# ziniuwan/maed

Measured on AMD Instinct MI355X. Metric: video-clips/sec (BxT frames) train step, higher is better.
Workload: dtype bf16

## Files before the change

### include/maed_hip.h

```cpp
#ifndef MAED_HIP_H
#define MAED_HIP_H

#include <stddef.h>
#include <stdint.h>

#ifdef __cplusplus
extern "C" {
#endif

typedef enum { MAED_F32 = 0, MAED_BF16 = 1,
               MAED_F32X3 = 2, MAED_F32X6 = 3,
               MAED_F32X1 = 4 } maed_dtype;

typedef enum {
    MAED_OK = 0,
    MAED_ERR_ARG = -1,
    MAED_ERR_SHAPE = -2,
    MAED_ERR_ALIGN = -3,
    MAED_ERR_LAUNCH = -4,
    MAED_ERR_UNSUPPORTED = -5
} maed_status;

typedef enum {
    MAED_EPI_STORE = 0,
// ... 17 lines not shown

const char* maed_last_error(void);
int maed_version(void);

typedef enum {
    MAED_OPT_F32_MATMUL = 0,
    MAED_OPT_SIDE_STREAM = 1,
    MAED_OPT_TN_TARGET_WGS = 2,
    MAED_OPT_ABLATE = 3,
    MAED_OPT_GN_BWD_ONEPASS = 4,
    MAED_OPT_F32_BWD_X1 = 5,
    MAED_OPT_ST_FUSED = 6,
    MAED_OPT_CONV3X3_ROWS_WGS = 7,
    MAED_OPT_STEM_WGRAD_WGS = 8,
    MAED_OPT_LBS_FRAMES = 9,
    MAED_OPT_TN_DMA = 10,
    MAED_OPT_X3_PLANES = 11,
    MAED_OPT_X3_PLANES_LN = 12,
    MAED_OPT_SK = 13,
    MAED_OPT_SK_GRID = 14,
    MAED_OPT_TN_SK = 15,
    MAED_OPT_CONV3X3_NARROW_WGS = 16,
    MAED_OPT_CONV3X3_FRAME = 17,
    MAED_OPT_COUNT
} maed_option;
int maed_init(int device);
int maed_device_faults(void);
int maed_device_faults_clear(void);
int maed_set_option(int key, int value);
int maed_get_option(int key);

int maed_layernorm_fwd(const float* x, int64_t x_row_stride, const float* gamma, const float* beta,
                       void* y, int dtype, float* mean, float* rstd,
                       int64_t rows, int C, float eps, void* stream);
int maed_layernorm_bwd(const void* dy, int dtype, const float* x, int64_t x_row_stride,
                       const float* gamma, const float* mean, const float* rstd,
                       const float* dres_in, float* dx_out, void* dx_twin, float* dgamma, float* dbeta,
                       int64_t rows, int C, void* stream);

int maed_gemm_nt(const void* A, int64_t lda, const void* B, int64_t ldb,
                 int64_t M, int64_t N, int64_t K, int dtype, int epilogue,
                 const float* bias, void* out, int64_t ldo, void* out2,
                 const void* aux, int64_t ldaux, int splitk, int impl, void* stream);

int maed_gemm_nt_planes(const void* a_hi, const void* a_lo, int64_t lda, const void* b_hi, const void* b_lo, int64_t ldb, int64_t M, int64_t N, int64_t K,
                        int epilogue, const float* bias, void* out, int64_t ldo, void* out2_bf16, const void* aux, int64_t ldaux, void* out_hi, void* out_lo,
// ... 157 lines not shown
int maed_groupnorm_fwd_twin(const void* x, const void* residual, const float* gamma, const float* beta, void* y, double* sums,
                            uint8_t* relu_mask, int N, int HW, int C, float eps, int relu, int sums_zeroed, void* twin_x, void* twin_y, void* stream);
#define MAED_GN_SYNC_WORDS 80
int maed_groupnorm_bwd(const void* x, const uint8_t* relu_mask, const void* dy, const double* sums, const float* gamma, const float* beta,
                       void* dx, void* dres, float* dgamma, float* dbeta, float* ab_scratch, int N, int HW, int C, float eps,
                       int relu, int dtype, int ab_zeroed, uint32_t* frame_sync, void* aux_stream, void* stream);
typedef struct { const float* ab; float* dgamma; float* dbeta; int N; int C; } maed_gn_affine_item;
int maed_gn_affine_grad_batch(const maed_gn_affine_item* items, int count, void* stream);

int maed_maxpool3s2_same_fwd(const void* x, void* y, uint8_t* idx, int N, int H, int W, int C, int dtype, void* stream);
int maed_maxpool3s2_same_bwd(const void* dy, const uint8_t* idx, void* dx, int N, int H, int W, int C, int dtype, void* stream);
int maed_gn_relu_maxpool3s2_fwd(const void* x, const float* gamma, const float* beta, void* y, uint8_t* idx, double* sums, int N, int H, int W, int C, float eps,
                                int dtype, int sums_zeroed, void* stream);
int maed_groupnorm_dual_fwd(const void* x, const float* gamma, const float* beta, double* sums, const void* res, const float* gamma2, const float* beta2,
                            double* sums2, void* y, uint8_t* relu_mask, int N, int HW, int C, float eps, float eps2, int dtype, int sums_zeroed,
                            int sums2_zeroed, void* stream);

int maed_stem_input(const float* x, void* y, int N, int C, int H, int W, int pad_top, int pad_bottom, int pad_left, int pad_right, int c_stride, int dtype,
                    void* stream);

int maed_conv3x3_wgrad_rows64_scratch_floats(int F, int H, int W, int Cin, int Cout);
int maed_conv3x3_wgrad_rows64(const void* dy, const void* x, float* dW, void* scratch, int F, int H, int W, int dtype, void* stream);

int maed_stem7x7s2_supported(int H, int W);
int maed_stem7x7s2_fwd(const void* xp, const void* w, void* wimg, void* y, double* gn_sums, int F, int H, int W, int dtype, void* stream);
int maed_stem7x7s2_wgrad_scratch_floats(int F, int H, int W);
int maed_stem7x7s2_wgrad(const void* dy, const void* xp, float* dW, void* scratch, int F, int H, int W, int dtype, void* stream);

int maed_subsample2_fwd(const void* x, void* y, int F, int H, int W, int C, int dtype, void* stream);
int maed_subsample2_bwd(const void* g, void* dx, int F, int H, int W, int C, int dtype, void* stream);

typedef struct { const float* src; void* dst_c; void* dst_t; int32_t rows, cols, tile0, tiles_n; } maed_wt_entry;
int maed_weight_refresh(const void* table, int n_entries, int n_tiles, int dtype, void* stream);

int maed_adam_step(float* p, const float* g, float* m, float* v, void* shadow_bf16, int64_t n,
                   float lr, float beta1, float beta2, float eps, float weight_decay,
                   float bias_corr1, float bias_corr2, float gscale, void* stream);
int maed_adam_step_dev(float* p, const float* g, float* m, float* v, void* shadow_bf16, int64_t n, const maed_train_state* state,
                       float beta1, float beta2, float eps, float weight_decay, float gscale, void* stream);

#define MAED_COMM_ID_BYTES 128
int maed_comm_load(const char* librccl_path);
int maed_comm_unique_id(void* id128);
int maed_comm_init(int rank, int world, const void* unique_id);
int maed_comm_allreduce_async(void* buf, size_t n, int dtype, void* compute_stream);
int maed_comm_wait(void* compute_stream);
// ... 60 lines not shown
```

### maed_amd/_lib.py

```python
import ctypes as C
import os

HERE = os.path.dirname(os.path.abspath(__file__))
LIB_PATH = os.environ.get("MAED_HIP_LIB") or os.path.join(HERE, "libmaed_hip.so")

F32, BF16 = 0, 1
F32X3, F32X6, F32X1 = 2, 3, 4
EPI_STORE, EPI_GELU, EPI_RESID_F32, EPI_MUL_DGELU, EPI_ATOMIC_F32, EPI_STORE_F32, EPI_TANH, EPI_ADD = range(8)
IMPL_AUTO, IMPL_VALU, IMPL_MFMA = 0, 1, 2
IMPL_MFMA_256 = 6
IMPL_MFMA_LONG = 5
IMPL_MFMA_SK = 10
IMPL_X3, IMPL_X6, IMPL_X1 = 7, 8, 9
(OPT_F32_MATMUL, OPT_SIDE_STREAM, OPT_TN_TARGET_WGS, OPT_ABLATE, OPT_GN_BWD_ONEPASS, OPT_F32_BWD_X1, OPT_ST_FUSED, OPT_CONV3X3_ROWS_WGS, OPT_STEM_WGRAD_WGS,
 OPT_LBS_FRAMES, OPT_TN_DMA, OPT_X3_PLANES, OPT_X3_PLANES_LN, OPT_SK, OPT_SK_GRID, OPT_TN_SK, OPT_CONV3X3_NARROW_WGS, OPT_CONV3X3_FRAME) = range(18)

vp, i64, i32, f32 = C.c_void_p, C.c_int64, C.c_int, C.c_float


class GnAffineItem(C.Structure):
    _fields_ = [("ab", C.c_void_p), ("dgamma", C.c_void_p), ("dbeta", C.c_void_p), ("N", C.c_int), ("C", C.c_int)]


class BlockDims(C.Structure):
    _fields_ = [("F", i32), ("P", i32), ("C", i32), ("H", i32), ("T", i32), ("hidden", i32),
                ("dtype", i32), ("impl", i32), ("eps", f32)]


_PARAM_FIELDS = ["ln1_g", "ln1_b", "ln2_g", "ln2_b", "w_qkv", "w_ts", "w_proj", "w_fc1", "w_fc2",
                 "b_qkv", "b_ts", "b_proj", "b_fc1", "b_fc2", "wt_qkv", "wt_ts", "wt_proj", "wt_fc1", "wt_fc2"]
_GRAD_FIELDS = _PARAM_FIELDS[:14]


class BlockParams(C.Structure):
    _fields_ = [(n, vp) for n in _PARAM_FIELDS]


class BlockGrads(C.Structure):
# ... 89 lines not shown
    "maed_comm_init": (i32, [i32, i32, vp]),
    "maed_comm_allreduce_async": (i32, [vp, C.c_size_t, i32, vp]),
    "maed_comm_wait": (i32, [vp]),
    "maed_comm_world": (i32, []),
    "maed_comm_destroy": (i32, []),
    "maed_conv3x3_fwd": (i32, [vp, vp, vp, vp, i32, i32, i32, i32, i32, i32, i32, i32, i32, i32, vp, i32, i32, vp, vp]),
    "maed_conv1x1_fwd": (i32, [vp, i64, vp, i64, i64, i32, i32, vp, i64, i32, vp, i32, vp]),
    "maed_conv3x3_tapmask": (i32, [vp, i32, i32, i32, vp]),
    "maed_conv3x3_s2_dgrad": (i32, [vp, vp, vp, vp, i32, i32, i32, i32, i32, i32, i32, i32, i32, i32, vp]),
    "maed_conv3x3_s2_tables": (i32, [vp, vp, i32, i32, i32, i32, i32, i32, i32, vp]),
    "maed_conv3x3_s2_wgrad": (i32, [vp, vp, vp, vp, vp, vp, i32, i32, i32, i32, i32, i32, i32, i32, vp]),
    "maed_conv3x3_wgrad": (i32, [vp, vp, vp, vp, vp, i32, i32, i32, i32, i32, i32, vp]),
    "maed_eval_pose_errors": (i32, [vp, vp, i32, i32, vp, vp, vp, vp, vp]),
    "maed_similarity_transform": (i32, [vp, vp, i32, i32, vp, vp]),
    "maed_eval_accel": (i32, [vp, vp, i32, i32, vp, vp]),
    "maed_eval_vertex_error": (i32, [vp, vp, i32, i32, vp, vp]),
    "maed_maxpool3s2_same_fwd": (i32, [vp, vp, vp, i32, i32, i32, i32, i32, vp]),
    "maed_maxpool3s2_same_bwd": (i32, [vp, vp, vp, i32, i32, i32, i32, i32, vp]),
    "maed_gn_relu_maxpool3s2_fwd": (i32, [vp, vp, vp, vp, vp, vp, i32, i32, i32, i32, f32, i32, i32, vp]),
    "maed_groupnorm_dual_fwd": (i32, [vp, vp, vp, vp, vp, vp, vp, vp, vp, vp, i32, i32, i32, f32, f32, i32, i32, i32, vp]),
    "maed_stem_input": (i32, [vp, vp, i32, i32, i32, i32, i32, i32, i32, i32, i32, i32, vp]),
    "maed_conv3x3_wgrad_rows64_scratch_floats": (i32, [i32, i32, i32, i32, i32]),
    "maed_conv3x3_wgrad_rows64": (i32, [vp, vp, vp, vp, i32, i32, i32, i32, vp]),
    "maed_stem7x7s2_supported": (i32, [i32, i32]),
    "maed_stem7x7s2_fwd": (i32, [vp, vp, vp, vp, vp, i32, i32, i32, i32, vp]),
    "maed_stem7x7s2_wgrad_scratch_floats": (i32, [i32, i32, i32]),
    "maed_stem7x7s2_wgrad": (i32, [vp, vp, vp, vp, i32, i32, i32, i32, vp]),
    "maed_subsample2_fwd": (i32, [vp, vp, i32, i32, i32, i32, i32, vp]),
    "maed_subsample2_bwd": (i32, [vp, vp, i32, i32, i32, i32, i32, vp]),
    "maed_weight_refresh": (i32, [vp, i32, i32, i32, vp]),
    "maed_adam_step": (i32, [vp, vp, vp, vp, vp, i64, f32, f32, f32, f32, f32, f32, f32, f32, vp]),
    "maed_adam_step_dev": (i32, [vp, vp, vp, vp, vp, i64, vp, f32, f32, f32, f32, f32, vp]),
    "maed_clip_preprocess_workspace": (C.c_size_t, [i32, i32, i32]),
    "maed_clip_preprocess": (i32, [vp, i64, vp, vp, vp, vp, i32, i32, i32, i32, C.POINTER(f32), i32, i32, vp, vp, C.c_size_t, vp]),
    "maed_render_mesh_workspace": (C.c_size_t, [i32, i32, i32, i32, i32, i32]),
    "maed_render_mesh": (i32, [vp, vp, vp, vp, vp, vp, vp, vp, vp, vp, vp, i32, i32, i32, i32, i32, C.POINTER(f32), f32, i32, vp, C.c_size_t, vp]),
    "maed_batchnorm_chunks": (i32, [i64]),
    "maed_batchnorm_stats": (i32, [vp, i64, i32, i32, vp, f32, vp, vp, vp, vp, vp, f32, vp]),
    "maed_batchnorm_finalize": (i32, [vp, i32, i32, C.c_double, f32, vp, vp, vp, vp, vp, f32, vp]),
    "maed_batchnorm_apply_fwd": (i32, [vp, vp, vp, vp, vp, vp, vp, vp, i64, i32, i32, i32, vp]),
    "maed_batchnorm_bwd_reduce": (i32, [vp, vp, vp, vp, vp, vp, vp, vp, vp, vp, vp, vp, i64, i32, i32, i32, vp]),
    "maed_batchnorm_bwd_apply": (i32, [vp, vp, vp, vp, vp, vp, vp, vp, vp, vp, vp, i64, i32, i32, i32, vp]),
    "maed_maxpool3s2p1_fwd": (i32, [vp, vp, vp, i32, i32, i32, i32, i32, vp]),
    "maed_maxpool3s2p1_bwd": (i32, [vp, vp, vp, i32, i32, i32, i32, i32, vp]),
    "maed_avgpool_fwd": (i32, [vp, vp, i32, i32, i32, i32, vp]),
    "maed_avgpool_bwd": (i32, [vp, vp, i32, i32, i32, i32, vp]),
# ... 24 lines not shown
        import torch
        if torch.cuda.is_available() and torch.cuda.is_initialized():
            _init_pending = False
            check(_lib.maed_init(torch.cuda.current_device()), "maed_init")
    return _lib


_OPTIONS = {
    OPT_F32_MATMUL: {"exact": 0, "0": 0, "bf16x3": 1, "1": 1, "bf16x6": 2, "2": 2}[os.environ.get("MAED_F32_MATMUL", "exact")],
    OPT_SIDE_STREAM: int(os.environ.get("MAED_WGRAD_SIDE_STREAM", "1") == "1"),
    OPT_TN_TARGET_WGS: int(os.environ.get("MAED_TN_TARGET_WGS", "0")),
    OPT_ABLATE: int(os.environ.get("MAED_GEMM_ABLATE", "0")),
    OPT_F32_BWD_X1: int(os.environ.get("MAED_F32_BWD", "") == "bf16x1"),
    OPT_ST_FUSED: int(os.environ.get("MAED_ST_FUSED", "1")),
    OPT_GN_BWD_ONEPASS: int(os.environ.get("MAED_GN_BWD_ONEPASS", "1")),
    OPT_CONV3X3_ROWS_WGS: 0 if os.environ.get("MAED_CONV3X3_WGRAD_ROWS", "1") == "0" else int(os.environ.get("MAED_CONV3X3_ROWS_WGS", "256")),
    OPT_STEM_WGRAD_WGS: int(os.environ.get("MAED_STEM_WGS", "512")),
    OPT_LBS_FRAMES: int(os.environ.get("MAED_LBS_FB", "0")),
    OPT_TN_DMA: int(os.environ.get("MAED_TN_DMA", "1")),
    OPT_X3_PLANES: int(os.environ.get("MAED_X3_PLANES", "6")),
    OPT_SK: int(os.environ.get("MAED_SK", "1")),
    OPT_SK_GRID: int(os.environ.get("MAED_SK_GRID", "0")),
    OPT_CONV3X3_FRAME: int(os.environ.get("MAED_CONV3X3_FRAME", "1")),
    OPT_CONV3X3_NARROW_WGS: int(os.environ.get("MAED_CONV3X3_NARROW_WGS", "0")),
    OPT_TN_SK: int(os.environ.get("MAED_TN_SK", "1")),
    OPT_X3_PLANES_LN: int(os.environ.get("MAED_X3_PLANES_LN", "0")),
}


def apply_options(handle):
    for k, v in _OPTIONS.items():
        if handle.maed_set_option(k, v) != 0:
            raise MaedHipError(f"maed_set_option({k}, {v}) failed")


def set_option(key, value):
    _OPTIONS[key] = int(value)
    if _lib is not None:
        check(_lib.maed_set_option(key, int(value)), "set_option")


def get_option(key):
    return _OPTIONS[key]


def check(rc, what=""):
# ... 12 lines not shown
```

### maed_amd/csrc/conv3x3_rows.hip

```cpp
#include "common.cuh"
#include "prof.h"

#define R3_ROWPX 66
#define R3_ROW_ELEMS (R3_ROWPX * 64)
#define R3_DY_ELEMS (64 * 64)
#define R3_THREADS 576
#define R3_RING 8
#define R3_NDY 4
#define R3_LDS_BYTES ((R3_RING * R3_ROW_ELEMS + R3_NDY * R3_DY_ELEMS) * 2)

__global__ __launch_bounds__(R3_THREADS, 1) void conv3x3_wgrad_rows64_kernel(const bf16* __restrict__ dy, const bf16* __restrict__ x, float* __restrict__ dW,
                                                                               float* __restrict__ partial, int H, int W, int n_rows, int rows_per_wg) {
    MAED_DYN_SHARED(unsigned short, smem);
    const int tid = threadIdx.x, lane = tid & 63, tap = __builtin_amdgcn_readfirstlane(tid >> 6), l31 = lane & 31, hi = lane >> 5, i16 = lane & 15;
    const int ky = tap / 3, kx = tap - 3 * ky;
    const int g0 = blockIdx.x * rows_per_wg;
    int g1 = g0 + rows_per_wg;
    if (g1 > n_rows) g1 = n_rows;
    if (g0 >= g1) return;
    for (int i = tid; i < R3_LDS_BYTES / 16; i += R3_THREADS) reinterpret_cast<uint4*>(smem)[i] = make_uint4(0u, 0u, 0u, 0u);
    __syncthreads();
    unsigned short* const ring = smem;
    unsigned short* const dyb = smem + R3_RING * R3_ROW_ELEMS;
    const int row_chunks = W * 8, n_instr = row_chunks >> 6;
// ... 91 lines not shown
    if (wgs == 0) return MAED_OK;
    static bool attr_set = false;
    if (!attr_set) { (void)hipFuncSetAttribute((const void*)conv3x3_wgrad_rows64_kernel, hipFuncAttributeMaxDynamicSharedMemorySize, 160 * 1024); attr_set = true; }
    hipLaunchKernelGGL(conv3x3_wgrad_rows64_kernel, dim3(wgs), dim3(R3_THREADS), R3_LDS_BYTES, stream, (const bf16*)dy, (const bf16*)x, dW, (float*)scratch, H, W, n_rows, per);
    if (scratch) maed_wgrad_slots_reduce((const float*)scratch, dW, wgs, 64 * 576, stream);
    MAED_CHECK_LAUNCH("conv3x3_wgrad(rows)");
    return MAED_OK;
}

extern "C" int maed_conv3x3_wgrad_rows64_scratch_floats(int F, int H, int W, int Cin, int Cout) {
    if (!maed_conv3x3_wgrad_rows64_ok(F, H, W, Cin, Cout)) return 0;
    int per = 0;
    return rows64_wgs(F * H, &per) * 64 * 576;
}

extern "C" int maed_conv3x3_wgrad_rows64(const void* dy, const void* x, float* dW, void* scratch, int F, int H, int W, int dtype, void* stream) {
    MAED_CHECK_ARG(dy && x && dW, MAED_ERR_ARG, "conv3x3_wgrad_rows64: null pointer");
    MAED_CHECK_ARG(dtype == MAED_BF16, MAED_ERR_UNSUPPORTED, "conv3x3_wgrad_rows64: bf16 only (dtype=%d)", dtype);
    MAED_CHECK_ARG(F > 0 && maed_conv3x3_wgrad_rows64_ok(F, H, W, 64, 64), MAED_ERR_SHAPE, "conv3x3_wgrad_rows64: needs W %% 8 == 0, 8 <= W <= 64 (F=%d H=%d W=%d)", F, H, W);
    MAED_CHECK_ARG(is_aligned(dy, 16) && is_aligned(x, 16) && is_aligned(scratch, 16), MAED_ERR_ALIGN, "conv3x3_wgrad_rows64: 16-B alignment");
    ProfScope prof__(PROF_TN_CONV, stream, 2.0 * (double)F * H * W * 64 * 576, 2.0 * (double)F * H * W * 128 + 36.0 * 64 * 64);
    return maed_conv3x3_wgrad_rows64_launch(dy, x, dW, scratch, F, H, W, (hipStream_t)stream);
}
```

### maed_amd/csrc/gemm_tn.hip

```cpp
#include "common.cuh"
#include "gemm_epilogue.cuh"
#include "gemm_x3.h"
#include "gemm_internal.h"
#include "prof.h"
#include <stdlib.h>

int maed_tn_splits(int tiles) {
    const int target = maed_opt(MAED_OPT_TN_TARGET_WGS);
    if (target > 0) return (target + tiles - 1) / tiles;
    if (tiles >= 32) return 512 / tiles > 0 ? 512 / tiles : 1;
    return (256 + tiles - 1) / tiles;
}
static int tn_remap() { return 1; }

bool maed_conv3x3_wgrad_rows64_ok(int F, int H, int W, int Cin, int Cout);
int maed_conv3x3_wgrad_rows64_launch(const void* dy, const void* x, float* dW, void* scratch, int F, int H, int W, hipStream_t stream);

#define TN_BM 64
#define TN_LD 72

__device__ __forceinline__ uint32_t perm_lo(uint32_t a, uint32_t b) { return __builtin_amdgcn_perm(b, a, 0x05040100u); }
__device__ __forceinline__ uint32_t perm_hi(uint32_t a, uint32_t b) { return __builtin_amdgcn_perm(b, a, 0x07060302u); }

struct TnConv { const uint16_t* tapmask; const bf16* zero_page; int Cin, Wimg;
                const int* rowtab = nullptr; };

template <bool CONV, bool S2 = false>
__global__ __launch_bounds__(256, 2) void gemm_tn_mfma_bf16_kernel(const bf16* __restrict__ Y, int64_t ldy, const bf16* __restrict__ X,
                                                                   int64_t ldx, int64_t M, int N, int K, float* __restrict__ dW,
                                                                   int64_t ldw, float* __restrict__ dbias, int tiles_k, int mtiles_per_split,
                                                                   TnConv cv, int remap
#ifdef MAED_GEMM_ABLATE
                                                                   , int ablate
#endif
                                                                   ) {
#ifndef MAED_GEMM_ABLATE
    constexpr int ablate = 0;
#endif
    __shared__ __attribute__((aligned(16))) unsigned short lds[2][2][128 * TN_LD];
// ... 275 lines not shown
extern "C" int maed_conv3x3_wgrad(const void* dy, const void* x, const void* tapmask, const void* zero_page, float* dW, int F, int H, int W, int Cin,
                                  int Cout, int dtype, void* stream) {
    MAED_CHECK_ARG(dy && x && tapmask && zero_page && dW, MAED_ERR_ARG, "conv3x3_wgrad: null pointer");
    const double es__ = (dtype == MAED_BF16) ? 2.0 : 4.0;
    ProfScope prof__(PROF_TN_CONV, stream, 2.0 * (double)F * H * W * Cout * 9 * Cin, es__ * (double)F * H * W * ((double)Cout + Cin) + 36.0 * (double)Cout * Cin);
    const int np_call = maed_x3_take_dtype(dtype);
    MAED_CHECK_ARG(dtype == MAED_BF16 || dtype == MAED_F32, MAED_ERR_ARG, "conv3x3_wgrad: bad dtype %d", dtype);
    const int64_t M = (int64_t)F * H * W;
    const int N = Cout, K = 9 * Cin;
    if (dtype == MAED_F32) {
        const int np = np_call ? np_call : maed_x3_planes();
        MAED_CHECK_ARG(np, MAED_ERR_UNSUPPORTED, "conv3x3_wgrad: f32 needs the split-bf16 matmul mode (maed_set_option(MAED_OPT_F32_MATMUL, 1 or 2))");
        MAED_CHECK_ARG(M > 0 && Cin % 4 == 0 && Cout % 4 == 0, MAED_ERR_SHAPE, "conv3x3_wgrad(f32): Cin / Cout must be multiples of 4 (Cin=%d Cout=%d)", Cin, Cout);
        MAED_CHECK_ARG(is_aligned(dy, 16) && is_aligned(x, 16) && is_aligned(tapmask, 16), MAED_ERR_ALIGN, "conv3x3_wgrad: 16-B alignment");
        const X3TnConv cv{(const uint16_t*)tapmask, Cin, W};
        MAED_PROPAGATE(maed_gemm_tn_x3_launch(np, dy, (int64_t)Cout, x, (int64_t)Cin, M, N, K, dW, (int64_t)K, nullptr, &cv, 0, (hipStream_t)stream));
        MAED_CHECK_LAUNCH("conv3x3_wgrad(x3)");
        return MAED_OK;
    }
    if (maed_conv3x3_wgrad_rows64_ok(F, H, W, Cin, Cout)) {
        MAED_CHECK_ARG(is_aligned(dy, 16) && is_aligned(x, 16), MAED_ERR_ALIGN, "conv3x3_wgrad: 16-B alignment");
        return maed_conv3x3_wgrad_rows64_launch(dy, x, dW, nullptr, F, H, W, (hipStream_t)stream);
    }
    MAED_CHECK_ARG(M > 0 && M % TN_BM == 0, MAED_ERR_SHAPE, "conv3x3_wgrad: F*H*W = %lld must be a multiple of 64", (long long)M);
    MAED_CHECK_ARG(Cin % 8 == 0 && Cout % 8 == 0 && Cin < (1 << 20) && W + 1 < (1 << 10), MAED_ERR_SHAPE, "conv3x3_wgrad: need Cin, Cout multiples of 8 (Cin=%d Cout=%d)", Cin, Cout);
    MAED_CHECK_ARG(is_aligned(dy, 16) && is_aligned(x, 16) && is_aligned(tapmask, 16) && is_aligned(zero_page, 16), MAED_ERR_ALIGN, "conv3x3_wgrad: 16-B alignment");
    const int tn = (N + 127) / 128, tk = (K + 127) / 128;
    const int nmt = (int)(M / TN_BM);
    int splits = maed_tn_splits(tn * tk);
    if (splits > (nmt + 3) / 4) splits = (nmt + 3) / 4;
    if (splits < 1) splits = 1;
    const int per = (nmt + splits - 1) / splits;
    const int z = (nmt + per - 1) / per;
    hipLaunchKernelGGL(gemm_tn_mfma_bf16_kernel<true>, dim3(tn * tk, 1, z), dim3(256), 0, (hipStream_t)stream, (const bf16*)dy, (int64_t)Cout,
                       (const bf16*)x, (int64_t)Cin, M, N, K, dW, (int64_t)K, (float*)nullptr, tk, per,
                       TnConv{(const uint16_t*)tapmask, (const bf16*)zero_page, Cin, W}, tn_remap()
#ifdef MAED_GEMM_ABLATE
                       , 0
#endif
                       );
    MAED_CHECK_LAUNCH("conv3x3_wgrad");
    return MAED_OK;
}
```

### maed_amd/csrc/options.hip

```cpp
#include "common.cuh"
#include "gemm_x3.h"
#include <atomic>
#include <string.h>

static std::atomic<int> g_opt[MAED_OPT_COUNT] = {
    {0},
    {1},
    {0},
    {0},
    {1},
    {0},
    {1},
    {256},
    {512},
    {0},
    {1},
    {6},
    {0},
    {1},
    {0},
    {1},
    {0},
    {1},
};

extern "C" int maed_init(int device) {
#ifndef MAED_HOSTSIM
    hipDeviceProp_t prop;
    if (hipGetDeviceProperties(&prop, device) != hipSuccess) { (void)hipGetLastError(); maed_set_error("init: no HIP device %d", device); return MAED_ERR_ARG; }
    if (!strstr(prop.gcnArchName, "gfx950")) {
        maed_set_error("init: device %d is %s; libmaed_hip is built for gfx950 (MI355X) only", device, prop.gcnArchName);
        return MAED_ERR_UNSUPPORTED;
    }
#else
    (void)device;
#endif
    (void)maed_fault_word();
#ifndef MAED_HOSTSIM
    if (maed_init_runtime() != MAED_OK) { maed_set_error("init: could not create the library's side streams / event rings"); return MAED_ERR_LAUNCH; }
#endif
    return MAED_OK;
}

static std::atomic<uint32_t*> g_fault{nullptr};
static std::atomic<int> g_fault_told{0};
// ... 26 lines not shown
                       "NaN-poisoned, the one-pass GroupNorm backward and the fused attentive addition now run as their multi-launch forms", who, *(volatile uint32_t*)w);
    return true;
}
extern "C" int maed_device_faults(void) {
    uint32_t* w = g_fault.load(std::memory_order_acquire);
    const int n = w ? (int)*(volatile uint32_t*)w : 0;
    if (n > 0)
        maed_set_error("%d frame-barrier timeout(s) on this device (workgroups of a frame were not co-resident: shared GPU / preemption); the affected results were "
                       "NaN-poisoned, the one-pass GroupNorm backward and the fused attentive addition run as their multi-launch forms from the next call on", n);
    return n;
}
extern "C" int maed_device_faults_clear(void) { uint32_t* w = g_fault.load(std::memory_order_acquire); if (w) *(volatile uint32_t*)w = 0; g_fault_told.store(0); return MAED_OK; }

extern "C" int maed_set_option(int key, int value) {
    MAED_CHECK_ARG(key >= 0 && key < MAED_OPT_COUNT, MAED_ERR_ARG, "set_option: unknown option %d", key);
    if (key == MAED_OPT_F32_MATMUL) MAED_CHECK_ARG(value >= 0 && value <= 2, MAED_ERR_ARG, "set_option: MAED_OPT_F32_MATMUL takes 0 (exact), 1 (bf16x3) or 2 (bf16x6)");
    if (key == MAED_OPT_TN_TARGET_WGS) MAED_CHECK_ARG(value == 0 || value >= 64, MAED_ERR_ARG, "set_option: MAED_OPT_TN_TARGET_WGS must be 0 (heuristic) or >= 64");
    if (key == MAED_OPT_CONV3X3_ROWS_WGS || key == MAED_OPT_STEM_WGRAD_WGS) MAED_CHECK_ARG(value >= 0 && value <= 65535, MAED_ERR_ARG, "set_option: workgroup count out of range");
    if (key == MAED_OPT_LBS_FRAMES) MAED_CHECK_ARG(value == 0 || value == 4 || value == 8 || value == 16, MAED_ERR_ARG, "set_option: MAED_OPT_LBS_FRAMES takes 0 (auto), 4, 8 or 16");
    if (key == MAED_OPT_X3_PLANES) MAED_CHECK_ARG(value == 0 || (value >= 2 && value <= 7 && value != 3), MAED_ERR_ARG, "set_option: MAED_OPT_X3_PLANES takes 0 (fp32 operands) or a kernel variant 2, 4, 5, 6, 7");
    if (key == MAED_OPT_SK) MAED_CHECK_ARG(value >= 0 && value <= 3, MAED_ERR_ARG, "set_option: MAED_OPT_SK takes 0 (off), 1 (heuristic), 2 (no K cuts) or 3 (always)");
    if (key == MAED_OPT_TN_SK) MAED_CHECK_ARG(value == 0 || value == 1, MAED_ERR_ARG, "set_option: MAED_OPT_TN_SK takes 0 or 1");
    if (key == MAED_OPT_SK_GRID) MAED_CHECK_ARG(value >= 0 && value <= 512, MAED_ERR_ARG, "set_option: MAED_OPT_SK_GRID takes 0 (one workgroup per CU) or a workgroup count <= 512");
    g_opt[key].store(value, std::memory_order_relaxed);
    return MAED_OK;
}

extern "C" int maed_get_option(int key) {
    if (key < 0 || key >= MAED_OPT_COUNT) { maed_set_error("get_option: unknown option %d", key); return MAED_ERR_ARG; }
    return g_opt[key].load(std::memory_order_relaxed);
}

int maed_opt(int key) { return g_opt[key].load(std::memory_order_relaxed); }

int maed_x3_planes(void) {
    const int v = maed_opt(MAED_OPT_F32_MATMUL);
    return v == 1 ? 2 : v == 2 ? 3 : 0;
}
```

### maed_amd/ops.py

```python
import ctypes as C
import math
import os
import threading
import weakref

import numpy as _np

import torch

from . import _lib as L
from ._lib import BF16, F32, check

WEIGHT_EPOCH = 0


def bump_weight_epoch():
    global WEIGHT_EPOCH
    WEIGHT_EPOCH += 1


def on_library_device(t):
    return t.is_cuda or (SIM_MODULE_PATHS and L._lib is not None and L._lib.maed_version() < 0)


# ... 1242 lines not shown


def _tapmask(N, H, W, device):
    key = (N, H, W, str(device))
    if key not in _TAPMASKS:
        n = (N * H * W + 63) // 64 * 64
        m = _aligned_bytes(2 * n, device)
        check(L.lib().maed_conv3x3_tapmask(_p(m), N, H, W, _stream()), "conv3x3_tapmask")
        _TAPMASKS[key] = m
    return _TAPMASKS[key]


def conv3x3_wgrad(dy, x, out=None, prec=None):
    N, I, H, W = x.shape
    O = dy.shape[1]
    dW = torch.zeros(O, 3, 3, I, dtype=torch.float32, device=x.device) if out is None else out
    if x.dtype == torch.bfloat16:
        nb = L.lib().maed_conv3x3_wgrad_rows64_scratch_floats(N, H, W, I, O)
        if nb > 0:
            scratch = torch.empty(nb, dtype=torch.float32, device=x.device)
            check(L.lib().maed_conv3x3_wgrad_rows64(_p(dy), _p(x), _p(dW), _p(scratch), N, H, W, dt_code(x.dtype), _stream()), "conv3x3_wgrad_rows64")
            _keep_alive_on_stream(scratch)
            return dW
    check(L.lib().maed_conv3x3_wgrad(_p(dy), _p(x), _p(_tapmask(N, H, W, x.device)), _p(_zero_page(x.device)), _p(dW), N, H, W, I, O,
                                     mm_code(x.dtype, prec), _stream()), "conv3x3_wgrad")
    return dW


_S2_TABLES = {}


def conv3x3_s2_wgrad(dy, x, pad_top, pad_left, out=None):
    N, I, H, W = x.shape
    O, Ho, Wo = dy.shape[1:]
    key = (N, H, W, Ho, Wo, pad_top, pad_left, str(x.device))
    if key not in _S2_TABLES:
        n = (N * Ho * Wo + 63) // 64 * 64
        mask, rows = _aligned_bytes(2 * n, x.device), _aligned_bytes(4 * n, x.device)
        check(L.lib().maed_conv3x3_s2_tables(_p(mask), _p(rows), N, H, W, pad_top, pad_left, Ho, Wo, _stream()), "conv3x3_s2_tables")
        _S2_TABLES[key] = (mask, rows)
    mask, rows = _S2_TABLES[key]
    dW = torch.zeros(O, 3, 3, I, dtype=torch.float32, device=x.device) if out is None else out
    check(L.lib().maed_conv3x3_s2_wgrad(_p(dy), _p(x), _p(mask), _p(rows), _p(_zero_page(x.device)), _p(dW), N, H, W, I, O, Ho, Wo, dt_code(x.dtype), _stream()),
          "conv3x3_s2_wgrad")
    return dW


class Conv3x3Fn(torch.autograd.Function):

    @staticmethod
    def forward(ctx, x, w, stride, wt=None, dw=None, gn_sums=None, prec=None):
        x32, w32 = shadow_of(x), shadow_of(w)
        assert (x32 is None) == (w32 is None), "Conv3x3Fn: activation and weight must both (or neither) have fp32 shadows"
        x = x.contiguous(memory_format=torch.channels_last)
        ctx.save_for_backward(x, w)
        ctx.stride, ctx.wt, ctx.dw, ctx.prec = stride, wt, dw, prec
        w_taps = (w if w32 is None else w32).permute(0, 2, 3, 1)
# ... 344 lines not shown
```

Measured before the change: 417.4.

## Add tap-parallel conv3x3 weight-gradient kernel for stride 1 and 2

Adds a new bf16 conv3x3 weight-gradient kernel where each of nine wavefronts owns one filter tap. Row bands of dy and x are staged once into LDS via DMA in a multi-stage pipeline and reused across all taps with MFMA 32x32x16. Partial sums are written per chunk and reduced afterwards. It is enabled by default for stride-1 shapes the rows64 path does not cover, and for stride-2 convolutions. This is meant to replace the generic tapmask and s2 table kernels. In exchange it adds scratch memory and a reduction pass.

After: 424.0, median of 6. 1.02x the previous value.

```diff
diff --git a/include/maed_hip.h b/include/maed_hip.h
--- a/include/maed_hip.h
+++ b/include/maed_hip.h
@@ -63,6 +63,7 @@
     MAED_OPT_TN_SK = 15,
     MAED_OPT_CONV3X3_NARROW_WGS = 16,
     MAED_OPT_CONV3X3_FRAME = 17,
+    MAED_OPT_CONV3X3_WGRAD_TAPS = 18,
     MAED_OPT_COUNT
 } maed_option;
 int maed_init(int device);
@@ -266,6 +267,10 @@
 int maed_conv3x3_wgrad_rows64_scratch_floats(int F, int H, int W, int Cin, int Cout);
 int maed_conv3x3_wgrad_rows64(const void* dy, const void* x, float* dW, void* scratch, int F, int H, int W, int dtype, void* stream);
 
+int maed_conv3x3_wgrad_taps_scratch_floats(int F, int H, int W, int Cin, int Cout, int stride, int Ho, int Wo);
+int maed_conv3x3_wgrad_taps(const void* dy, const void* x, const void* zero_page, float* dW, void* scratch, int F, int H, int W, int Cin, int Cout, int stride,
+                            int pad_top, int pad_left, int Ho, int Wo, int dtype, void* stream);
+
 int maed_stem7x7s2_supported(int H, int W);
 int maed_stem7x7s2_fwd(const void* xp, const void* w, void* wimg, void* y, double* gn_sums, int F, int H, int W, int dtype, void* stream);
 int maed_stem7x7s2_wgrad_scratch_floats(int F, int H, int W);
diff --git a/maed_amd/_lib.py b/maed_amd/_lib.py
--- a/maed_amd/_lib.py
+++ b/maed_amd/_lib.py
@@ -13,7 +13,7 @@
 IMPL_MFMA_SK = 10
 IMPL_X3, IMPL_X6, IMPL_X1 = 7, 8, 9
 (OPT_F32_MATMUL, OPT_SIDE_STREAM, OPT_TN_TARGET_WGS, OPT_ABLATE, OPT_GN_BWD_ONEPASS, OPT_F32_BWD_X1, OPT_ST_FUSED, OPT_CONV3X3_ROWS_WGS, OPT_STEM_WGRAD_WGS,
- OPT_LBS_FRAMES, OPT_TN_DMA, OPT_X3_PLANES, OPT_X3_PLANES_LN, OPT_SK, OPT_SK_GRID, OPT_TN_SK, OPT_CONV3X3_NARROW_WGS, OPT_CONV3X3_FRAME) = range(18)
+ OPT_LBS_FRAMES, OPT_TN_DMA, OPT_X3_PLANES, OPT_X3_PLANES_LN, OPT_SK, OPT_SK_GRID, OPT_TN_SK, OPT_CONV3X3_NARROW_WGS, OPT_CONV3X3_FRAME, OPT_CONV3X3_WGRAD_TAPS) = range(19)
 
 vp, i64, i32, f32 = C.c_void_p, C.c_int64, C.c_int, C.c_float
 
@@ -149,6 +149,8 @@
     "maed_stem_input": (i32, [vp, vp, i32, i32, i32, i32, i32, i32, i32, i32, i32, i32, vp]),
     "maed_conv3x3_wgrad_rows64_scratch_floats": (i32, [i32, i32, i32, i32, i32]),
     "maed_conv3x3_wgrad_rows64": (i32, [vp, vp, vp, vp, i32, i32, i32, i32, vp]),
+    "maed_conv3x3_wgrad_taps_scratch_floats": (i32, [i32, i32, i32, i32, i32, i32, i32, i32]),
+    "maed_conv3x3_wgrad_taps": (i32, [vp, vp, vp, vp, vp, i32, i32, i32, i32, i32, i32, i32, i32, i32, i32, i32, vp]),
     "maed_stem7x7s2_supported": (i32, [i32, i32]),
     "maed_stem7x7s2_fwd": (i32, [vp, vp, vp, vp, vp, i32, i32, i32, i32, vp]),
     "maed_stem7x7s2_wgrad_scratch_floats": (i32, [i32, i32, i32]),
@@ -219,6 +221,7 @@
     OPT_SK: int(os.environ.get("MAED_SK", "1")),
     OPT_SK_GRID: int(os.environ.get("MAED_SK_GRID", "0")),
     OPT_CONV3X3_FRAME: int(os.environ.get("MAED_CONV3X3_FRAME", "1")),
+    OPT_CONV3X3_WGRAD_TAPS: int(os.environ.get("MAED_CONV3X3_WGRAD_TAPS", "1")),
     OPT_CONV3X3_NARROW_WGS: int(os.environ.get("MAED_CONV3X3_NARROW_WGS", "0")),
     OPT_TN_SK: int(os.environ.get("MAED_TN_SK", "1")),
     OPT_X3_PLANES_LN: int(os.environ.get("MAED_X3_PLANES_LN", "0")),
diff --git a/maed_amd/csrc/conv3x3_rows.hip b/maed_amd/csrc/conv3x3_rows.hip
--- a/maed_amd/csrc/conv3x3_rows.hip
+++ b/maed_amd/csrc/conv3x3_rows.hip
@@ -137,3 +137,202 @@
     ProfScope prof__(PROF_TN_CONV, stream, 2.0 * (double)F * H * W * 64 * 576, 2.0 * (double)F * H * W * 128 + 36.0 * 64 * 64);
     return maed_conv3x3_wgrad_rows64_launch(dy, x, dW, scratch, F, H, W, (hipStream_t)stream);
 }
+
+#define T9_THREADS 576
+#define T9_MAXDY 4
+#define T9_MAXX 8
+#define T9_MAX_SLOTS 1280
+
+struct TapsGeo {
+    int H, W, Ho, Wo, Cin, Cout, s2, pt, pl;
+    int R, ipf, n_items;
+    int P, ksteps, DS, XP, XS, nst;
+    int per, chunks, cib, cob;
+};
+
+#define T9_WAIT(n_) switch (n_) { case 1: MAED_WAIT_VMCNT(1); break; case 2: MAED_WAIT_VMCNT(2); break; case 3: MAED_WAIT_VMCNT(3); break; case 4: MAED_WAIT_VMCNT(4); break; \
+    case 5: MAED_WAIT_VMCNT(5); break; case 6: MAED_WAIT_VMCNT(6); break; case 7: MAED_WAIT_VMCNT(7); break; case 8: MAED_WAIT_VMCNT(8); break; case 9: MAED_WAIT_VMCNT(9); break; \
+    case 10: MAED_WAIT_VMCNT(10); break; case 11: MAED_WAIT_VMCNT(11); break; case 12: MAED_WAIT_VMCNT(12); break; default: MAED_WAIT_VMCNT0(); }
+
+__global__ __launch_bounds__(T9_THREADS, 1) void conv3x3_wgrad_taps_kernel(const bf16* __restrict__ dy, const bf16* __restrict__ x, const bf16* __restrict__ zero,
+                                                                             float* __restrict__ dW, float* __restrict__ partial, TapsGeo g) {
+    MAED_DYN_SHARED(unsigned short, smem);
+    const int tid = threadIdx.x, lane = tid & 63, tap = __builtin_amdgcn_readfirstlane(tid >> 6), l31 = lane & 31, hi = lane >> 5, i16 = lane & 15;
+    const int ky = tap / 3, kx = tap - 3 * ky;
+    const int i0 = blockIdx.x * g.per;
+    int i1 = i0 + g.per;
+    if (i1 > g.n_items) i1 = g.n_items;
+    if (i0 >= i1) return;
+    const int cb = blockIdx.y / g.cib, ib = blockIdx.y - cb * g.cib;
+    const int P = g.P, ndi = g.DS >> 3, nxi = g.XS >> 3, stage_elems = (g.DS + g.XS) * 64;
+
+    int dyrel[T9_MAXDY], dyrow[T9_MAXDY], xrel[T9_MAXX], xrow[T9_MAXX];
+    int n_mine = 0;
+#pragma unroll
+    for (int q = 0; q < T9_MAXDY; ++q) {
+        const int s = (tap + 9 * q) * 8 + (lane >> 3), r = s / P, c = s - r * P, ch = (lane & 7) ^ (((s >> 1) & 1) << 2);
+        dyrow[q] = (c < g.Wo && r < g.R) ? r : (1 << 20);
+        dyrel[q] = ((r * g.Wo + c) * g.Cout + cb * 64) * 2 + ch * 16;
+        n_mine += (tap + 9 * q < ndi) ? 1 : 0;
+    }
+#pragma unroll
+    for (int q = 0; q < T9_MAXX; ++q) {
+        const int u = (tap + 9 * q) * 8 + (lane >> 3), ch = (lane & 7) ^ (((u >> 1) & 1) << 2);
+        int ro, col;
+        bool ok;
+        if (!g.s2) { const int rr = u / P; ro = rr - 1; col = u - rr * P - 1; ok = rr < g.R + 2; }
+        else { const int ph = u / g.XP, v = u - ph * g.XP, rr = v / P; ro = 2 * rr + (ph >> 1); col = 2 * (v - rr * P) + (ph & 1) - g.pl; ok = rr < g.R + 1; }
+        xrow[q] = (ok && (unsigned)col < (unsigned)g.W) ? ro : (1 << 20);
+        xrel[q] = ((ro * g.W + col) * g.Cin + ib * 64) * 2 + ch * 16;
+        n_mine += (tap + 9 * q < nxi) ? 1 : 0;
+    }
+    n_mine = __builtin_amdgcn_readfirstlane(n_mine);
+#define T9_ISSUE(it_, st_) { const int it__ = (it_), f__ = it__ / g.ipf, y0__ = (it__ - f__ * g.ipf) * g.R, yb__ = g.s2 ? 2 * y0__ - g.pt : y0__; \
+        unsigned short* const sb__ = smem + (st_) * stage_elems; \
+        const char* const dyb__ = (const char*)dy + ((int64_t)f__ * g.Ho + y0__) * g.Wo * g.Cout * 2; \
+        const char* const xb__ = (const char*)x + ((int64_t)f__ * g.H + yb__) * g.W * g.Cin * 2; \
+        _Pragma("unroll") for (int q = 0; q < T9_MAXDY; ++q) if (tap + 9 * q < ndi) { \
+            const char* s__ = (unsigned)(y0__ + dyrow[q]) < (unsigned)g.Ho ? dyb__ + dyrel[q] : (const char*)zero; \
+            MAED_LDS_DMA16_PTR(s__, sb__ + (tap + 9 * q) * 512); } \
+        _Pragma("unroll") for (int q = 0; q < T9_MAXX; ++q) if (tap + 9 * q < nxi) { \
+            const char* s__ = (unsigned)(yb__ + xrow[q]) < (unsigned)g.H ? xb__ + xrel[q] : (const char*)zero; \
+            MAED_LDS_DMA16_PTR(s__, sb__ + g.DS * 64 + (tap + 9 * q) * 512); } }
+
+    f32x16_t acc[2][2];
+#pragma unroll
+    for (int r = 0; r < 16; ++r) { acc[0][0][r] = 0.f; acc[0][1][r] = 0.f; acc[1][0][r] = 0.f; acc[1][1][r] = 0.f; }
+    const int toff = g.s2 ? ((ky & 1) * 2 + (kx & 1)) * g.XP + (ky >> 1) * P + (kx >> 1) : ky * P + kx;
+    const int prow = 4 * hi + (i16 >> 2), pcol = (lane & 16) + 4 * (i16 & 3);
+    const int swa = ((prow >> 1) & 1) << 2, swb = (((prow + toff) >> 1) & 1) << 2;
+    const int a_off0 = prow * 64 + ((((pcol >> 3) ^ swa) << 3) | (pcol & 7)), a_off1 = prow * 64 + (((((pcol + 32) >> 3) ^ swa) << 3) | (pcol & 7));
+    const int b_off0 = (prow + toff) * 64 + ((((pcol >> 3) ^ swb) << 3) | (pcol & 7)), b_off1 = (prow + toff) * 64 + (((((pcol + 32) >> 3) ^ swb) << 3) | (pcol & 7));
+
+    const int ahead = g.nst - 1;
+    T9_ISSUE(i0, 0);
+    if (ahead > 1 && i0 + 1 < i1) T9_ISSUE(i0 + 1, 1);
+    int st = 0;
+    for (int it = i0; it < i1; ++it) {
+        if (ahead > 1 && it + 1 < i1) { T9_WAIT(n_mine) } else { MAED_WAIT_VMCNT0(); }
+        __syncthreads();
+        if (it + ahead < i1) { int sn = st + ahead; if (sn >= g.nst) sn -= g.nst; T9_ISSUE(it + ahead, sn); }
+        const unsigned short* da = smem + st * stage_elems;
+        const unsigned short* xb = da + g.DS * 64;
+        union Frag { bf16x8_t v; uint2 u[2]; };
+        Frag pa0, pa1, pb0, pb1, qa0, qa1, qb0, qb1;
+#define T9_FRAG(dst_, base_, s_, off_) { auto lo__ = MAED_DS_READ_TR16((base_) + (s_) * 1024 + (off_)); auto hi__ = MAED_DS_READ_TR16((base_) + (s_) * 1024 + 512 + (off_)); \
+            __builtin_memcpy(&dst_.u[0], &lo__, 8); __builtin_memcpy(&dst_.u[1], &hi__, 8); }
+#define T9_LOAD(p_, s_) { T9_FRAG(p_##a0, da, s_, a_off0) T9_FRAG(p_##a1, da, s_, a_off1) T9_FRAG(p_##b0, xb, s_, b_off0) T9_FRAG(p_##b1, xb, s_, b_off1) }
+#define T9_MFMA(p_) { acc[0][0] = __builtin_amdgcn_mfma_f32_32x32x16_bf16(p_##a0.v, p_##b0.v, acc[0][0], 0, 0, 0); \
+            acc[0][1] = __builtin_amdgcn_mfma_f32_32x32x16_bf16(p_##a0.v, p_##b1.v, acc[0][1], 0, 0, 0); \
+            acc[1][0] = __builtin_amdgcn_mfma_f32_32x32x16_bf16(p_##a1.v, p_##b0.v, acc[1][0], 0, 0, 0); \
+            acc[1][1] = __builtin_amdgcn_mfma_f32_32x32x16_bf16(p_##a1.v, p_##b1.v, acc[1][1], 0, 0, 0); }
+        T9_LOAD(p, 0)
+        int s = 0;
+        for (; s + 2 <= g.ksteps; s += 2) {
+            T9_LOAD(q, s + 1)
+            __builtin_amdgcn_sched_barrier(0);
+            T9_MFMA(p)
+            __builtin_amdgcn_sched_barrier(0);
+            { const int sn = s + 2 < g.ksteps ? s + 2 : s; T9_LOAD(p, sn) }
+            __builtin_amdgcn_sched_barrier(0);
+            T9_MFMA(q)
+            __builtin_amdgcn_sched_barrier(0);
+        }
+        if (s < g.ksteps) T9_MFMA(p)
+#undef T9_MFMA
+#undef T9_LOAD
+#undef T9_FRAG
+        if (++st == g.nst) st = 0;
+    }
+#undef T9_ISSUE
+    const size_t ld = (size_t)9 * g.Cin;
+    float* const base = (partial ? partial + (size_t)blockIdx.x * g.Cout * ld : dW) + (size_t)cb * 64 * ld + tap * g.Cin + ib * 64;
+#pragma unroll
+    for (int a = 0; a < 2; ++a)
+#pragma unroll
+        for (int bt = 0; bt < 2; ++bt) {
+            float* d = base + 32 * bt + l31;
+#pragma unroll
+            for (int r = 0; r < 16; ++r) {
+                float* e = d + (size_t)(32 * a + (r & 3) + 8 * (r >> 2) + 4 * hi) * ld;
+                if (partial) *e = acc[a][bt][r]; else atomicAdd(e, acc[a][bt][r]);
+            }
+        }
+}
+
+static bool taps_geo(int F, int H, int W, int Cin, int Cout, int stride, int pt, int pl, int Ho, int Wo, TapsGeo* out) {
+    const int opt = maed_opt(MAED_OPT_CONV3X3_WGRAD_TAPS);
+    if (opt <= 0 || F < 1 || H < 1 || W < 1 || Ho < 1 || Wo < 1 || Cin < 64 || Cout < 64 || Cin % 64 || Cout % 64) return false;
+    if (stride == 1) { if (Ho != H || Wo != W || maed_conv3x3_wgrad_rows64_ok(F, H, W, Cin, Cout)) return false; }
+    else if (stride == 2) { if (Ho != (H + 1) / 2 || Wo != (W + 1) / 2 || pt < 0 || pt > 1 || pl < 0 || pl > 1) return false; }
+    else return false;
+    if ((int64_t)H * W * Cin * 2 >= (1ll << 30) || (int64_t)Ho * Wo * Cout * 2 >= (1ll << 30) || (int64_t)Cout * 9 * Cin >= (1ll << 28)) return false;
+    const int64_t M = (int64_t)F * Ho * Wo;
+    if (opt == 1 && M < 4096 && M % 64 == 0) return false;
+    TapsGeo g{};
+    g.H = H; g.W = W; g.Ho = Ho; g.Wo = Wo; g.Cin = Cin; g.Cout = Cout; g.s2 = stride == 2; g.pt = pt; g.pl = pl;
+    g.P = g.s2 ? Wo + 1 : Wo + 2;
+    int rmax = 0;
+    for (int R = 1; R <= Ho; ++R) {
+        const int DS = (R * g.P + 15) / 16 * 16, XP = (DS + g.P + 1 + 7) / 8 * 8, XS = g.s2 ? 4 * XP : (DS + 2 * g.P + 2 + 7) / 8 * 8;
+        if (DS > T9_MAXDY * 72 || XS > T9_MAXX * 72 || 2 * (DS + XS) > T9_MAX_SLOTS) break;
+        rmax = R;
+    }
+    if (rmax == 0) return false;
+    g.ipf = (Ho + rmax - 1) / rmax;
+    g.R = (Ho + g.ipf - 1) / g.ipf;
+    g.ipf = (Ho + g.R - 1) / g.R;
+    if ((int64_t)F * g.ipf >= (1ll << 30)) return false;
+    g.n_items = F * g.ipf;
+    g.DS = (g.R * g.P + 15) / 16 * 16; g.ksteps = g.DS / 16;
+    g.XP = (g.DS + g.P + 1 + 7) / 8 * 8;
+    g.XS = g.s2 ? 4 * g.XP : (g.DS + 2 * g.P + 2 + 7) / 8 * 8;
+    g.nst = 3 * (g.DS + g.XS) <= T9_MAX_SLOTS ? 3 : 2;
+    g.cib = Cin / 64; g.cob = Cout / 64;
+    if ((int64_t)g.cib * g.cob > 65535) return false;
+    const int wgs = maed_opt(MAED_OPT_SIDE_STREAM) ? 64 : 256;
+    int chunks = opt > 2 ? opt - 2 : (wgs + g.cib * g.cob - 1) / (g.cib * g.cob);
+    if (chunks > g.n_items) chunks = g.n_items;
+    g.per = (g.n_items + chunks - 1) / chunks;
+    g.chunks = (g.n_items + g.per - 1) / g.per;
+    *out = g;
+    return true;
+}
+
+bool maed_conv3x3_wgrad_taps_ok(int F, int H, int W, int Cin, int Cout, int stride, int pad_top, int pad_left, int Ho, int Wo) {
+    TapsGeo g;
+    return taps_geo(F, H, W, Cin, Cout, stride, pad_top, pad_left, Ho, Wo, &g);
+}
+
+int maed_conv3x3_wgrad_taps_launch(const void* dy, const void* x, const void* zero_page, float* dW, void* scratch, int F, int H, int W, int Cin, int Cout, int stride,
+                                   int pad_top, int pad_left, int Ho, int Wo, hipStream_t stream) {
+    TapsGeo g;
+    if (!taps_geo(F, H, W, Cin, Cout, stride, pad_top, pad_left, Ho, Wo, &g)) { maed_set_error("conv3x3_wgrad_taps: shape not covered"); return MAED_ERR_SHAPE; }
+    static bool attr_set = false;
+    if (!attr_set) { (void)hipFuncSetAttribute((const void*)conv3x3_wgrad_taps_kernel, hipFuncAttributeMaxDynamicSharedMemorySize, 160 * 1024); attr_set = true; }
+    const size_t lds_bytes = (size_t)g.nst * (g.DS + g.XS) * 128;
+    hipLaunchKernelGGL(conv3x3_wgrad_taps_kernel, dim3(g.chunks, g.cib * g.cob), dim3(T9_THREADS), lds_bytes, stream, (const bf16*)dy, (const bf16*)x,
+                       (const bf16*)zero_page, dW, (float*)scratch, g);
+    if (scratch) maed_wgrad_slots_reduce((const float*)scratch, dW, g.chunks, Cout * 9 * Cin, stream);
+    MAED_CHECK_LAUNCH("conv3x3_wgrad(taps)");
+    return MAED_OK;
+}
+
+extern "C" int maed_conv3x3_wgrad_taps_scratch_floats(int F, int H, int W, int Cin, int Cout, int stride, int Ho, int Wo) {
+    TapsGeo g;
+    if (!taps_geo(F, H, W, Cin, Cout, stride, 0, 0, Ho, Wo, &g)) return 0;
+    const int64_t n = (int64_t)g.chunks * Cout * 9 * Cin;
+    return n < (1ll << 31) ? (int)n : 0;
+}
+
+extern "C" int maed_conv3x3_wgrad_taps(const void* dy, const void* x, const void* zero_page, float* dW, void* scratch, int F, int H, int W, int Cin, int Cout,
+                                       int stride, int pad_top, int pad_left, int Ho, int Wo, int dtype, void* stream) {
+    MAED_CHECK_ARG(dy && x && zero_page && dW, MAED_ERR_ARG, "conv3x3_wgrad_taps: null pointer");
+    MAED_CHECK_ARG(dtype == MAED_BF16, MAED_ERR_UNSUPPORTED, "conv3x3_wgrad_taps: bf16 only (dtype=%d)", dtype);
+    MAED_CHECK_ARG(maed_conv3x3_wgrad_taps_ok(F, H, W, Cin, Cout, stride, pad_top, pad_left, Ho, Wo), MAED_ERR_SHAPE,
+                   "conv3x3_wgrad_taps: shape not covered (F=%d H=%d W=%d Cin=%d Cout=%d stride=%d pads %d/%d Ho=%d Wo=%d, option %d)", F, H, W, Cin, Cout, stride,
+                   pad_top, pad_left, Ho, Wo, maed_opt(MAED_OPT_CONV3X3_WGRAD_TAPS));
+    MAED_CHECK_ARG(is_aligned(dy, 16) && is_aligned(x, 16) && is_aligned(zero_page, 16) && is_aligned(scratch, 16), MAED_ERR_ALIGN, "conv3x3_wgrad_taps: 16-B alignment");
+    ProfScope prof__(PROF_TN_CONV, stream, 2.0 * (double)F * Ho * Wo * Cout * 9 * Cin, 2.0 * ((double)F * Ho * Wo * Cout + (double)F * H * W * Cin) + 36.0 * (double)Cout * Cin);
+    return maed_conv3x3_wgrad_taps_launch(dy, x, zero_page, dW, scratch, F, H, W, Cin, Cout, stride, pad_top, pad_left, Ho, Wo, (hipStream_t)stream);
+}
diff --git a/maed_amd/csrc/gemm_tn.hip b/maed_amd/csrc/gemm_tn.hip
--- a/maed_amd/csrc/gemm_tn.hip
+++ b/maed_amd/csrc/gemm_tn.hip
@@ -15,6 +15,9 @@
 
 bool maed_conv3x3_wgrad_rows64_ok(int F, int H, int W, int Cin, int Cout);
 int maed_conv3x3_wgrad_rows64_launch(const void* dy, const void* x, float* dW, void* scratch, int F, int H, int W, hipStream_t stream);
+bool maed_conv3x3_wgrad_taps_ok(int F, int H, int W, int Cin, int Cout, int stride, int pad_top, int pad_left, int Ho, int Wo);
+int maed_conv3x3_wgrad_taps_launch(const void* dy, const void* x, const void* zero_page, float* dW, void* scratch, int F, int H, int W, int Cin, int Cout, int stride,
+                                   int pad_top, int pad_left, int Ho, int Wo, hipStream_t stream);
 
 #define TN_BM 64
 #define TN_LD 72
@@ -336,6 +339,10 @@
         MAED_CHECK_ARG(is_aligned(dy, 16) && is_aligned(x, 16), MAED_ERR_ALIGN, "conv3x3_wgrad: 16-B alignment");
         return maed_conv3x3_wgrad_rows64_launch(dy, x, dW, nullptr, F, H, W, (hipStream_t)stream);
     }
+    if (maed_conv3x3_wgrad_taps_ok(F, H, W, Cin, Cout, 1, 0, 0, H, W)) {
+        MAED_CHECK_ARG(is_aligned(dy, 16) && is_aligned(x, 16) && is_aligned(zero_page, 16), MAED_ERR_ALIGN, "conv3x3_wgrad: 16-B alignment");
+        return maed_conv3x3_wgrad_taps_launch(dy, x, zero_page, dW, nullptr, F, H, W, Cin, Cout, 1, 0, 0, H, W, (hipStream_t)stream);
+    }
     MAED_CHECK_ARG(M > 0 && M % TN_BM == 0, MAED_ERR_SHAPE, "conv3x3_wgrad: F*H*W = %lld must be a multiple of 64", (long long)M);
     MAED_CHECK_ARG(Cin % 8 == 0 && Cout % 8 == 0 && Cin < (1 << 20) && W + 1 < (1 << 10), MAED_ERR_SHAPE, "conv3x3_wgrad: need Cin, Cout multiples of 8 (Cin=%d Cout=%d)", Cin, Cout);
     MAED_CHECK_ARG(is_aligned(dy, 16) && is_aligned(x, 16) && is_aligned(tapmask, 16) && is_aligned(zero_page, 16), MAED_ERR_ALIGN, "conv3x3_wgrad: 16-B alignment");
diff --git a/maed_amd/csrc/options.hip b/maed_amd/csrc/options.hip
--- a/maed_amd/csrc/options.hip
+++ b/maed_amd/csrc/options.hip
@@ -21,6 +21,7 @@
     {0},
     {1},
     {0},
+    {1},
     {1},
 };
 
@@ -93,6 +94,7 @@
     if (key == MAED_OPT_SK) MAED_CHECK_ARG(value >= 0 && value <= 3, MAED_ERR_ARG, "set_option: MAED_OPT_SK takes 0 (off), 1 (heuristic), 2 (no K cuts) or 3 (always)");
     if (key == MAED_OPT_TN_SK) MAED_CHECK_ARG(value == 0 || value == 1, MAED_ERR_ARG, "set_option: MAED_OPT_TN_SK takes 0 or 1");
     if (key == MAED_OPT_SK_GRID) MAED_CHECK_ARG(value >= 0 && value <= 512, MAED_ERR_ARG, "set_option: MAED_OPT_SK_GRID takes 0 (one workgroup per CU) or a workgroup count <= 512");
+    if (key == MAED_OPT_CONV3X3_WGRAD_TAPS) MAED_CHECK_ARG(value >= 0 && value <= 2 + 65535, MAED_ERR_ARG, "set_option: MAED_OPT_CONV3X3_WGRAD_TAPS takes 0, 1, 2 or 2 + a chunk count");
     g_opt[key].store(value, std::memory_order_relaxed);
     return MAED_OK;
 }
diff --git a/maed_amd/ops.py b/maed_amd/ops.py
--- a/maed_amd/ops.py
+++ b/maed_amd/ops.py
@@ -1288,17 +1288,37 @@
             check(L.lib().maed_conv3x3_wgrad_rows64(_p(dy), _p(x), _p(dW), _p(scratch), N, H, W, dt_code(x.dtype), _stream()), "conv3x3_wgrad_rows64")
             _keep_alive_on_stream(scratch)
             return dW
+        if _conv3x3_wgrad_taps(dy, x, dW, 1, 0, 0):
+            return dW
     check(L.lib().maed_conv3x3_wgrad(_p(dy), _p(x), _p(_tapmask(N, H, W, x.device)), _p(_zero_page(x.device)), _p(dW), N, H, W, I, O,
                                      mm_code(x.dtype, prec), _stream()), "conv3x3_wgrad")
     return dW
 
 
+def _conv3x3_wgrad_taps(dy, x, dW, stride, pad_top, pad_left):
+    N, I, H, W = x.shape
+    O, Ho, Wo = dy.shape[1:]
+    nb = L.lib().maed_conv3x3_wgrad_taps_scratch_floats(N, H, W, I, O, stride, Ho, Wo)
+    if nb <= 0:
+        return False
+    scratch = torch.empty(nb, dtype=torch.float32, device=x.device)
+    check(L.lib().maed_conv3x3_wgrad_taps(_p(dy), _p(x), _p(_zero_page(x.device)), _p(dW), _p(scratch), N, H, W, I, O, stride, pad_top, pad_left, Ho, Wo,
+                                          dt_code(x.dtype), _stream()), "conv3x3_wgrad_taps")
+    _keep_alive_on_stream(scratch)
+    return True
+
+
 _S2_TABLES = {}
 
 
 def conv3x3_s2_wgrad(dy, x, pad_top, pad_left, out=None):
     N, I, H, W = x.shape
     O, Ho, Wo = dy.shape[1:]
+    if x.dtype == torch.bfloat16 and pad_top in (0, 1) and pad_left in (0, 1):
+        dW = torch.zeros(O, 3, 3, I, dtype=torch.float32, device=x.device) if out is None else out
+        if _conv3x3_wgrad_taps(dy, x, dW, 2, pad_top, pad_left):
+            return dW
+        out = dW
     key = (N, H, W, Ho, Wo, pad_top, pad_left, str(x.device))
     if key not in _S2_TABLES:
         n = (N * Ho * Wo + 63) // 64 * 64
```
